# wbw520/scouter

Hardware: AMD Instinct MI355X
Metric: images/sec training step (resnest26d+xSlot, 224^2, bs70) (higher is better)
Workload: dtype f32; 1 GPU; BASELINE configs[1]: ImageNet-10 resnest26d + positive xSlot, channel 2048, T=3, to_k_layer 3, power 2, 224x224, per-GPU batch 70, random init, AdamW lr 1e-4; precision=fp32, activation_storage=fp32, register_split_bf16x3_layers=16, global_batch=70, parallelism=dp1, step=zero_grad+fwd+loss+bwd(+allreduce)+adamw, launch=eager

## Files before the change

include/scouter_hip.h:

```cpp
#ifndef SCOUTER_HIP_H
#define SCOUTER_HIP_H
#include <stddef.h>
#ifdef __cplusplus
extern "C" {
#endif

#define SC_OK 0
#define SC_ERR_ARG (-1)
#define SC_ERR_LAUNCH (-2)
#define SC_ERR_UNSUPPORTED (-3)
#define SC_ERR_WORKSPACE (-4)

int scouter_abi_version(void);
const char* scouter_last_error(void);

int scouter_set_switch(const char* name, int value);
int scouter_get_switch(const char* name);

int scouter_resize_normalize_u8_f32(const unsigned char* const* srcs, const int* hw, unsigned char* tmp,
                                    const long* tmp_off, const float* lut, float* out, int B, int C, int max_h, int max_w,
                                    int out_h, int out_w, void* stream);

void scouter_prof_enable(int on);
int scouter_prof_collect(char* buf, int cap);
// ... 291 lines not shown
int scouter_conv2d_x3_tile(long M, int N, int tile_hint);
int scouter_conv2d_x3_partial_rows(long M, int N, int tile_hint);
int scouter_conv2d_x3_halo_partial_rows(int groups);
int scouter_conv2d_fwd_x3(const float* x, const void* w_planes_fwd, const float* bias, const float* addend, float* y,
                          double* bn_partial, int B, int H, int W, int Cin, int Cout, int kh, int kw, int pad, int groups,
                          int relu, int tile_hint, void* stream);
int scouter_conv2d_dgrad_x3_bnbwd(const float* dy, const void* w_planes_dgrad, const float* addend, float* dx, int B,
                                  int H, int W, int Cin, int Cout, int kh, int kw, int pad, int groups, int tile_hint,
                                  const void* relu_mask, const float* x1, const float* saved1, double* part1,
                                  const float* x2, const float* saved2, double* part2, void* stream);

size_t scouter_conv2d_wgrad_x3_workspace_bytes(int B, int H, int W, int Cin, int Cout, int plan_hint);
int scouter_conv2d_wgrad_x3(const float* x, const float* dy, float* dw, int B, int H, int W, int Cin, int Cout,
                            int plan_hint, void* ws, size_t ws_bytes, void* stream);

size_t scouter_bn_fold_row_bytes(void);
int scouter_bn_fold_multi(const void* table, int nrows, long total, void* stream);
int scouter_sa_gate_fwd_f32(const float* gap, const float* w1, const float* b1, const float* w2, const float* b2, float* a,
                            int B, int Cp, int A, void* stream);

int scouter_iadd_i64(long* p, long n, long v, void* stream);

int scouter_adamw_chunk_bytes(void);
int scouter_adamw_step_f32(const void* chunk_table, int nchunks, const float* grads, float* exp_avg,
                           float* exp_avg_sq, float lr, float beta1, float beta2, float eps, float weight_decay,
                           int step, void* stream);
int scouter_adamw_step_dev_f32(const void* chunk_table, int nchunks, const float* grads, float* exp_avg,
                               float* exp_avg_sq, const float* dyn, float beta1, float beta2, float eps,
                               float weight_decay, void* stream);

// ... 5 lines not shown
```

scouter_amd/csrc/abi_core.hip:

```cpp
#include "common.h"

#include <stdarg.h>
#include <stdlib.h>
#include <atomic>
#include <map>
#include <mutex>
#include <vector>

#define SCOUTER_ABI_VERSION 1

static thread_local char g_err[512] = "";
static thread_local hipError_t g_lds_err = hipSuccess;

void sc_set_error(const char* fmt, ...) {
    va_list ap;
    va_start(ap, fmt);
    vsnprintf(g_err, sizeof(g_err), fmt, ap);
    va_end(ap);
}

int sc_check_launch(const char* what) {
    hipError_t e = hipGetLastError();
    if (e == hipSuccess) e = g_lds_err;
    g_lds_err = hipSuccess;
    if (e != hipSuccess) {
        sc_set_error("%s: launch failed: %s", what, hipGetErrorString(e));
        return SC_ERR_LAUNCH;
    }
    return SC_OK;
}

extern "C" int scouter_abi_version(void) { return SCOUTER_ABI_VERSION; }
extern "C" const char* scouter_last_error(void) { return g_err; }

static const char* const g_switch_names[SC_SW_COUNT] = {"xwt", "bwt", "bhalo", "xslot_small", "xslot_bwd_halves",
                                                         "xslot_bwd_scratch", "pwp_bn", "pwp_resident"};
struct SwitchTable {
    std::atomic<int> v[SC_SW_COUNT] = {};
    SwitchTable() {
        static const char* const flags[] = {"SCOUTER_XWT", "SCOUTER_BWT", "SCOUTER_BHALO", "SCOUTER_XSLOT_SMALL",
                                            "SCOUTER_XSLOT_BWD_HALVES", "SCOUTER_XSLOT_BWD_SCRATCH"};
        for (int i = 0; i <= SC_SW_XSLOT_BWD_SCRATCH; ++i) {
            const int def = i != SC_SW_XSLOT_BWD_SCRATCH;
            const char* e = getenv(flags[i]);
            v[i] = e && e[0] == '1' - def ? !def : def;
        }
        int bn = 0, r = 0;
        const char* e = getenv("SCOUTER_PWP_PLAN_DEV");
        if (e && sscanf(e, "%d,%d", &bn, &r) == 2 && bn > 0 && r > 0) { v[SC_SW_PWP_BN] = bn; v[SC_SW_PWP_RESIDENT] = r; }
    }
};
static SwitchTable& switch_table() {
    static SwitchTable t;
    return t;
}
int sc_switch(ScSwitch s) { return switch_table().v[s].load(std::memory_order_relaxed); }

static int switch_index(const char* name) {
    for (int i = 0; name && i < SC_SW_COUNT; ++i)
        if (strcmp(name, g_switch_names[i]) == 0) return i;
    sc_set_error("unknown switch '%s'", name ? name : "(null)");
// ... 81 lines not shown
```

scouter_amd/csrc/common.h:

```cpp
#pragma once
#include <hip/hip_runtime.h>
#include <stdint.h>
#include <stdio.h>
#include <string.h>

#define SC_OK 0
#define SC_ERR_ARG (-1)
#define SC_ERR_LAUNCH (-2)
#define SC_ERR_UNSUPPORTED (-3)
#define SC_ERR_WORKSPACE (-4)

typedef float f32x4 __attribute__((ext_vector_type(4)));
typedef float f32x16 __attribute__((ext_vector_type(16)));

void sc_set_error(const char* fmt, ...);
int sc_check_launch(const char* what);

enum ScSwitch { SC_SW_XWT, SC_SW_BWT, SC_SW_BHALO, SC_SW_XSLOT_SMALL, SC_SW_XSLOT_BWD_HALVES, SC_SW_XSLOT_BWD_SCRATCH,
                SC_SW_PWP_BN, SC_SW_PWP_RESIDENT, SC_SW_COUNT };
int sc_switch(ScSwitch s);

void sc_dyn_lds(const void* kern, size_t bytes);

#define SC_REQUIRE(cond, ...)                 \
    do {                                      \
        if (!(cond)) {                        \
            sc_set_error(__VA_ARGS__);        \
            return SC_ERR_ARG;                \
        }                                     \
    } while (0)

#define SC_UNSUPPORTED(cond, ...)             \
    do {                                      \
        if (!(cond)) {                        \
// ... 160 lines not shown
```

scouter_amd/csrc/conv_common.h:

```cpp
#pragma once
#include "common.h"

struct ConvGeom {
    int B, H, W, C;
    int Ho, Wo;
    int N;
    int R, S, stride, pad, groups;
    int Cg, Ng;
    long M;
    int wrow, wtap;
    double inv_hw;
    float inv_wo, inv_ho;
};

inline int sc_conv_out(int in, int k, int s, int p) { return (in + 2 * p - k) / s + 1; }

inline bool sc_pixels_ok(int B, int H, int W) {
    return B > 0 && H > 0 && W > 0 && H <= (1 << 24) && W <= (1 << 24) && (long)B * H <= (1L << 36) / W;
}
inline bool sc_conv_args_ok(int B, int H, int W, int Cin, int Cout, int kh, int kw, int stride, int pad, int groups) {
    const int lim = 1 << 16;
    return kh > 0 && kw > 0 && kh < lim && kw < lim && stride > 0 && pad >= 0 && pad < lim && sc_pixels_ok(B, H, W) &&
           sc_pixels_ok(B, H + 2 * pad, W + 2 * pad) && Cin > 0 && Cout > 0 && Cin <= (1 << 20) && Cout <= (1 << 20) && groups > 0 &&
           Cin % groups == 0 && Cout % groups == 0 && (long)(Cin / groups) * Cout < (1L << 31) && H + 2 * pad >= kh &&
// ... 42 lines not shown
__device__ __forceinline__ int fast_div(int n, float inv) { return (int)(((float)n + 0.5f) * inv); }


__device__ __forceinline__ void wgrad_block_coords(int& tile, int& split) {
    const int T = gridDim.x, S = gridDim.y, S8 = S & ~7;
    const int L = blockIdx.x + T * blockIdx.y;
    tile = blockIdx.x;
    split = blockIdx.y;
    if (L < T * S8) {
        const int xcd = L & 7, idx = L >> 3;
        split = xcd + 8 * (idx / T);
        tile = idx % T;
    }
}

void sc_launch_slab_reduce(const float* part, float* dst, long n, int splits, long slab, hipStream_t st);

struct BnBwdFuse {
    const unsigned long long* mask;
    const float* x1; const float* sv1; double* part1;
    const float* x2; const float* sv2; double* part2;
    int io;
};

bool sc_xhalo_ok(const ConvGeom& g);
int sc_xhalo_partial_rows(int groups);
void sc_launch_xhalo(bool dgrad, const float* a, const void* w_planes, long w_plane_elems, const float* addend, float* dst,
                     double* bn_part, const ConvGeom& g, int relu, hipStream_t st, const BnBwdFuse& fz);

template <int NR>
struct EpiPre { f32x4 add[NR], x1[NR], x2[NR]; bool on; };
// ... 361 lines not shown
```

scouter_amd/csrc/conv_igemm.hip:

```cpp
#include "conv_common.h"
#include "conv_wgrad_bf16.h"
#include "conv_wgrad_taps.h"
#include "conv_wgrad_taps_x3.h"
#include "conv_wgrad_taps_bf16.h"
#include "conv_pw_persist.h"
#include "conv_pw_persist_x3.h"

#include <stdlib.h>
#include <type_traits>

#ifdef IGEMM_STAMPS
__device__ long long* g_igemm_stamps = nullptr;
extern "C" int scouter_dev_set_igemm_stamps(void* p) {
    return (int)hipMemcpyToSymbol(HIP_SYMBOL(g_igemm_stamps), &p, sizeof(p));
}
#define IG_STAMP(k) if (g_igemm_stamps && threadIdx.x == 0) { asm volatile("s_waitcnt lgkmcnt(0)" ::: "memory"); g_igemm_stamps[8L * blockIdx.x + (k)] = (long long)wall_clock64(); }
#else
#define IG_STAMP(k)
#endif

constexpr int BK = 32;
constexpr int LDK = BK + 4;

template <int BM, int BN, bool B_KC>
// ... 520 lines not shown
        for (; k + 96 < splits; k += 128) {
#pragma unroll
            for (int u = 0; u < 4; ++u) s4[u] += *(const f32x4*)(part + (long)(k + 32 * u) * slab + i);
        }
        for (; k < splits; k += 32) s4[0] += *(const f32x4*)(part + (long)k * slab + i);
    }
    red[lane][q] = (s4[0] + s4[1]) + (s4[2] + s4[3]);
    __syncthreads();
    if (lane == 0 && i < n) {
        f32x4 s = red[0][q];
        for (int k = 1; k < 32; ++k) s += red[k][q];
        *(f32x4*)(dst + i) = s;
    }
}

void sc_launch_slab_reduce(const float* part, float* dst, long n, int splits, long slab, hipStream_t st) {
    hipLaunchKernelGGL(slab_reduce_kernel, dim3(sc_cdiv(n / 4, 8)), dim3(256), 0, st, part, dst, n, splits, slab);
}

template <int BM, int BN, int WM, int WN, bool DGRAD, bool STRIDED, bool PW>
static void launch_igemm_s(const float* src, const float* w, const float* bias, const float* addend, float* dst,
                           double* bn_part, const ConvGeom& g, int relu, hipStream_t st, const BnBwdFuse& fz) {
    const int mtiles = sc_cdiv(g.M, BM), ntiles = g.Ng / BN;
    dim3 grid(mtiles * ntiles * g.groups);
    const ConvGeom gg = sc_with_reciprocals(g);
    if (DGRAD && fz.part1)
        hipLaunchKernelGGL((igemm_kernel<BM, BN, WM, WN, DGRAD, STRIDED, PW, DGRAD>), grid, dim3(256), 0, st, src, w, bias,
                           addend, dst, bn_part, gg, relu, mtiles, ntiles, fz);
    else
        hipLaunchKernelGGL((igemm_kernel<BM, BN, WM, WN, DGRAD, STRIDED, PW, false>), grid, dim3(256), 0, st, src, w, bias,
                           addend, dst, bn_part, gg, relu, mtiles, ntiles, fz);
}
// ... 348 lines not shown
extern "C" size_t scouter_conv2d_wgrad_workspace_bytes(int B, int H, int W, int Cin, int Cout, int kh, int kw,
                                                       int stride, int pad, int groups, int plan_hint) {
    if (groups <= 0 || Cin % groups || Cout % groups) return 0;
    ConvGeom g = wgrad_geom(B, H, W, Cin, Cout, kh, kw, stride, pad, groups);
    WgradPlan p = wgrad_plan(g, plan_hint);
    size_t need = p.splits <= 1 ? 0 : (size_t)p.splits * kh * kw * g.Cg * Cout * sizeof(float);
    if (plan_hint < 0 && wgrad_taps_geom_ok(g)) {
        const long tiles = (long)(g.Ng / (g.Ng % 64 == 0 ? 64 : 32)) * groups;
        long want = 1024 / tiles;
        if (want < 1) want = 1;
        long chunks = (g.M + BK - 1) / BK, cps = (chunks + want - 1) / want;
        if (cps < 8) cps = 8;
        const long splits = (g.M + cps * BK - 1) / (cps * BK);
        const size_t nt = splits > 1 ? (size_t)splits * 9 * g.Cg * Cout * sizeof(float) : 0;
        if (nt > need) need = nt;
    }
    return need;
}

extern "C" int scouter_conv2d_wgrad_f32(const float* x, const float* dy, float* dw, int B, int H, int W, int Cin,
                                        int Cout, int kh, int kw, int stride, int pad, int groups, int plan_hint,
                                        void* ws, size_t ws_bytes, void* stream) {
    SC_REQUIRE(x && dy && dw && B > 0, "conv2d_wgrad: null pointer or empty shape");
    SC_REQUIRE(groups > 0 && Cin % groups == 0 && Cout % groups == 0, "conv2d_wgrad: channels not divisible by groups");
    ConvGeom g = wgrad_geom(B, H, W, Cin, Cout, kh, kw, stride, pad, groups);
    SC_UNSUPPORTED(wgrad_entry_ok(g), "conv2d_wgrad: per-group channels must be multiples of 32");
    if (plan_hint < 0 && wgrad_taps_geom_ok(g)) {
        const int bn = g.Ng % 64 == 0 ? 64 : 32;
        const int co_tiles = g.Ng / bn;
        const long tiles = (long)co_tiles * groups;
// ... 17 lines not shown
                                 4.0 * ((double)B * H * W * Cin + (double)g.M * Cout));
                auto kern = bn == 64 ? xwgrad_taps_kernel<64> : xwgrad_taps_kernel<32>;
                sc_dyn_lds((const void*)kern, xlds);
                hipLaunchKernelGGL(kern, dim3((unsigned)tiles, (unsigned)splits), dim3(256), xlds, st, x, dy, out, g, co_tiles,
                                   pps, slab_t);
            } else {
                ScProfScope prof("wgrad_taps", st, 2.0 * g.M * Cout * g.Cg * 9,
                                 4.0 * ((double)B * H * W * Cin + (double)g.M * Cout));
                auto kern = bn == 64 ? wgrad_taps_kernel<64> : wgrad_taps_kernel<32>;
                sc_dyn_lds((const void*)kern, lds);
                hipLaunchKernelGGL(kern, dim3((unsigned)tiles, (unsigned)splits), dim3(256), lds, st, x, dy, out, g, co_tiles,
                                   pps, slab_t);
            }
            int rc = sc_check_launch("conv2d_wgrad_taps");
            if (rc) return rc;
            if (splits > 1) {
                ScProfScope prof2("slab_reduce", st, 0, 4.0 * (double)slab_t * (splits + 1));
                hipLaunchKernelGGL(slab_reduce_kernel, dim3(sc_cdiv(slab_t / 4, 8)), dim3(256), 0, st, (const float*)ws,
                                   dw, slab_t, splits, slab_t);
                rc = sc_check_launch("conv2d_wgrad_taps_reduce");
            }
            return rc;
        }
    }
    WgradPlan p = wgrad_plan(g, plan_hint);
    const long slab = (long)kh * kw * g.Cg * Cout;
    const size_t need = p.splits > 1 ? (size_t)p.splits * slab * sizeof(float) : 0;
    if (need > ws_bytes || (need && !ws)) {
        sc_set_error("conv2d_wgrad: workspace too small (%zu < %zu bytes)", ws_bytes, need);
        return SC_ERR_WORKSPACE;
    }
    hipStream_t st = (hipStream_t)stream;
    float* out = p.splits > 1 ? (float*)ws : dw;
    dim3 grid((unsigned)p.tiles, (unsigned)p.splits);
    static char wname[9][24];
    static const int wb[9][2] = {{128, 128}, {128, 64}, {128, 32}, {64, 128}, {64, 64}, {64, 32}, {32, 128}, {32, 64}, {32, 32}};
// ... 18 lines not shown
                               p.ci_tiles, p.co_tiles, p.pix_per_split, slab);                                     \
    } while (0)
    if (p.bm == 128 && p.bn == 128) WG(128, 128, 64, 64);
    else if (p.bm == 128 && p.bn == 64) WG(128, 64, 64, 32);
    else if (p.bm == 128 && p.bn == 32) WG(128, 32, 32, 32);
    else if (p.bm == 64 && p.bn == 128) WG(64, 128, 32, 64);
    else if (p.bm == 64 && p.bn == 64) WG(64, 64, 32, 32);
    else if (p.bm == 64 && p.bn == 32) WG(64, 32, 32, 32);
    else if (p.bm == 32 && p.bn == 128) WG(32, 128, 32, 32);
    else if (p.bm == 32 && p.bn == 64) WG(32, 64, 32, 32);
    else WG(32, 32, 32, 32);
#undef WG
    }
    rc = sc_check_launch("conv2d_wgrad");
    if (rc) return rc;
    if (p.splits > 1) {
        const long n = slab;
        ScProfScope prof2("slab_reduce", st, 0, 4.0 * (double)slab * (p.splits + 1));
        hipLaunchKernelGGL(slab_reduce_kernel, dim3(sc_cdiv(n / 4, 8)), dim3(256), 0, st, (const float*)ws, dw, n,
                           p.splits, slab);
        rc = sc_check_launch("conv2d_wgrad_reduce");
    }
    return rc;
}

extern "C" int scouter_conv2d_wgrad_bf16_io(const void* x, const void* dy, float* dw, int B, int H, int W, int Cin,
                                            int Cout, int kh, int kw, int stride, int pad, int groups, int plan_hint,
                                            void* ws, size_t ws_bytes, int io, void* stream) {
    SC_REQUIRE(x && dy && dw && B > 0, "conv2d_wgrad_bf16: null pointer or empty shape");
    SC_REQUIRE((io & ~(SC_IO_X_BF16 | SC_IO_R_BF16)) == 0, "conv2d_wgrad_bf16: unsupported io bits %d (x and dy may be bf16)", io);
    const bool xb = (io & SC_IO_X_BF16) != 0, db = (io & SC_IO_R_BF16) != 0;
    SC_REQUIRE(groups > 0 && Cin % groups == 0 && Cout % groups == 0, "conv2d_wgrad_bf16: channels not divisible by groups");
    ConvGeom g = wgrad_geom(B, H, W, Cin, Cout, kh, kw, stride, pad, groups);
    const int mode = wgrad_same_mode(g, 64);
    SC_UNSUPPORTED(wgrad_bf16_geom_ok(g), "conv2d_wgrad_bf16: shape not covered by the bf16 kernel");
    if (plan_hint < 0 && bwt_geom_ok(g, io)) {
        const int bn = g.Ng % 64 == 0 ? 64 : 32;
// ... 8 lines not shown
        const long slab_t = (long)9 * g.Cg * Cout;
        const size_t need_t = splits > 1 ? (size_t)splits * slab_t * sizeof(float) : 0;
        if (sc_switch(SC_SW_BWT) && need_t <= ws_bytes && (!need_t || ws)) {
            hipStream_t st = (hipStream_t)stream;
            float* out = splits > 1 ? (float*)ws : dw;
            const size_t blds = bwgrad_taps_lds_bytes(bn);
            {
            ScProfScope prof("bwgrad_taps<bf16>", st, 2.0 * g.M * Cout * g.Cg * 9, 2.0 * ((double)B * H * W * Cin + (double)g.M * Cout));
            auto kern = bn == 64 ? bwgrad_taps_kernel<64> : bwgrad_taps_kernel<32>;
            sc_dyn_lds((const void*)kern, blds);
            hipLaunchKernelGGL(kern, dim3((unsigned)tiles, (unsigned)splits), dim3(256), blds, st, (const unsigned short*)x,
                               (const unsigned short*)dy, out, g, co_tiles, pps, slab_t);
            }
            int rc = sc_check_launch("conv2d_wgrad_taps_bf16");
            if (rc) return rc;
            if (splits > 1) {
                ScProfScope prof2("slab_reduce", st, 0, 4.0 * (double)slab_t * (splits + 1));
                hipLaunchKernelGGL(slab_reduce_kernel, dim3(sc_cdiv(slab_t / 4, 8)), dim3(256), 0, st, (const float*)ws,
                                   dw, slab_t, splits, slab_t);
                rc = sc_check_launch("conv2d_wgrad_taps_bf16_reduce");
            }
            return rc;
        }
    }
    WgradPlan p = wgrad_plan(g, plan_hint, true, 64);
    const long slab = (long)kh * kw * g.Cg * Cout;
    const size_t need = p.splits > 1 ? (size_t)p.splits * slab * sizeof(float) : 0;
    if (need > ws_bytes || (need && !ws)) {
        sc_set_error("conv2d_wgrad_bf16: workspace too small (%zu < %zu bytes)", ws_bytes, need);
        return SC_ERR_WORKSPACE;
    }
    hipStream_t st = (hipStream_t)stream;
    float* out = p.splits > 1 ? (float*)ws : dw;
    dim3 grid((unsigned)p.tiles, (unsigned)p.splits);
    int rc;
    {
// ... 15 lines not shown
        else if (mode == 2) WGK((wgrad_bf16_kernel<BM_, BN_, WM_, WN_, 2, false, false>));                          \
        else if (xb && db) WGK((wgrad_bf16_kernel<BM_, BN_, WM_, WN_, 1, true, true>));                             \
        else if (xb) WGK((wgrad_bf16_kernel<BM_, BN_, WM_, WN_, 1, true, false>));                                  \
        else if (db) WGK((wgrad_bf16_kernel<BM_, BN_, WM_, WN_, 1, false, true>));                                  \
        else WGK((wgrad_bf16_kernel<BM_, BN_, WM_, WN_, 1, false, false>));                                         \
    } while (0)
    if (p.bm == 128 && p.bn == 128) WGH(128, 128, 64, 64);
    else if (p.bm == 128 && p.bn == 64) WGH(128, 64, 64, 32);
    else if (p.bm == 64 && p.bn == 128) WGH(64, 128, 32, 64);
    else WGH(64, 64, 32, 32);
#undef WGH
#undef WGK
    }
    rc = sc_check_launch("conv2d_wgrad_bf16");
    if (rc) return rc;
    if (p.splits > 1) {
        ScProfScope prof2("slab_reduce", st, 0, 4.0 * (double)slab * (p.splits + 1));
        hipLaunchKernelGGL(slab_reduce_kernel, dim3(sc_cdiv(slab / 4, 8)), dim3(256), 0, st, (const float*)ws, dw, slab,
                           p.splits, slab);
        rc = sc_check_launch("conv2d_wgrad_bf16_reduce");
    }
    return rc;
}
extern "C" int scouter_conv2d_wgrad_bf16(const float* x, const float* dy, float* dw, int B, int H, int W, int Cin,
                                         int Cout, int kh, int kw, int stride, int pad, int groups, int plan_hint,
                                         void* ws, size_t ws_bytes, void* stream) {
    return scouter_conv2d_wgrad_bf16_io(x, dy, dw, B, H, W, Cin, Cout, kh, kw, stride, pad, groups, plan_hint, ws, ws_bytes,
                                        0, stream);
}
```

scouter_amd/csrc/conv_planes.hip:

```cpp
#include "conv_common.h"

#include <type_traits>

typedef __bf16 bf16x8 __attribute__((ext_vector_type(8)));

#define LDS_PTR(p) ((__attribute__((address_space(3))) void*)(p))

__device__ __forceinline__ void dma16(__amdgpu_buffer_rsrc_t rs, char* lds, unsigned voff, int soff) {
    __builtin_amdgcn_raw_ptr_buffer_load_lds(rs, LDS_PTR(lds), 16, voff, soff, 0, 0);
}

__device__ __forceinline__ f32x16 mfma_bf16p(bf16x8 a, bf16x8 b, f32x16 c) {
    return __builtin_amdgcn_mfma_f32_32x32x16_bf16(a, b, c, 0, 0, 0);
}

#define split3 split3_bf16

template <int NP>
__global__ __launch_bounds__(256) void split_planes_kernel(const float* __restrict__ x, unsigned short* __restrict__ p,
                                                           long n4, long plane_elems) {
    for (long i = (long)blockIdx.x * blockDim.x + threadIdx.x; i < n4; i += (long)gridDim.x * blockDim.x) {
        const f32x4 v = *(const f32x4*)(x + i * 4);
        u16x4 h, m, l;
#pragma unroll
// ... 1096 lines not shown
        if (nplanes == 3) {
            if (bm == 128 && bn == 128) PWG(128, 128, 3);
            else if (bm == 128) PWG(128, 64, 3);
            else if (bn == 128) PWG(64, 128, 3);
            else PWG(64, 64, 3);
        } else {
            if (bm == 128 && bn == 128) PWG(128, 128, 1);
            else if (bm == 128) PWG(128, 64, 1);
            else if (bn == 128) PWG(64, 128, 1);
            else PWG(64, 64, 1);
        }
#undef PWG
    }
    int rc = sc_check_launch("conv2d_wgrad_planes");
    if (rc) return rc;
    if (splits > 1) {
        ScProfScope prof2("slab_reduce", st, 0, 4.0 * (double)slab * (splits + 1));
        sc_launch_slab_reduce((const float*)ws, dw, slab, splits, slab, st);
        rc = sc_check_launch("conv2d_wgrad_planes_reduce");
    }
    return rc;
}
```

scouter_amd/csrc/conv_x3.hip:

```cpp
#include "conv_common.h"

#include <stdlib.h>
#include <type_traits>

typedef __bf16 xbf16x8 __attribute__((ext_vector_type(8)));
typedef unsigned short xu16x8 __attribute__((ext_vector_type(8)));

#define X3_LDS_PTR(p) ((__attribute__((address_space(3))) void*)(p))

#ifndef X3_ABLATE
#define X3_ABLATE 0
#endif

__device__ __forceinline__ void x3_dma16(__amdgpu_buffer_rsrc_t rs, char* lds, unsigned voff, int soff) {
    __builtin_amdgcn_raw_ptr_buffer_load_lds(rs, X3_LDS_PTR(lds), 16, voff, soff, 0, 0);
}
__device__ __forceinline__ f32x16 x3_mfma(xbf16x8 a, xbf16x8 b, f32x16 c) {
    return __builtin_amdgcn_mfma_f32_32x32x16_bf16(a, b, c, 0, 0, 0);
}

template <int BM, int BN, int NWM, int NWN, int MINB, bool DGRAD, bool CONV>
__global__ __launch_bounds__(NWM * NWN * 64, MINB) void xgemm_kernel(const float* __restrict__ a_f32,
                                                                       const unsigned short* __restrict__ w_planes, long w_plane_elems,
                                                                       const float* __restrict__ bias, const float* __restrict__ addend,
// ... 594 lines not shown
        return SC_ERR_WORKSPACE;
    }
    hipStream_t st = (hipStream_t)stream;
    float* out = p.splits > 1 ? (float*)ws : dw;
    int rc;
    {
        ScProfScope prof("xwgrad<bf16x3>", st, 2.0 * g.M * Cout * Cin, 4.0 * g.M * (Cin + Cout));
        constexpr int LDS = 2 * 3 * (128 + 128) * 40 * 2;
        auto kern = xwgrad_kernel<0>;
        sc_dyn_lds((const void*)kern, LDS);
        hipLaunchKernelGGL(kern, dim3((unsigned)p.tiles, (unsigned)p.splits), dim3(256), LDS, st, x, dy, out, g, p.ci_tiles,
                           p.co_tiles, p.pix_per_split, slab);
        rc = sc_check_launch("conv2d_wgrad_x3");
    }
    if (rc) return rc;
    if (p.splits > 1) {
        ScProfScope prof2("slab_reduce", st, 0, 4.0 * (double)slab * (p.splits + 1));
        sc_launch_slab_reduce((const float*)ws, dw, slab, p.splits, slab, st);
        rc = sc_check_launch("conv2d_wgrad_x3_reduce");
    }
    return rc;
}
```

scouter_amd/graph.py:

```python
import torch

from . import kernels as K


class GraphedTrainStep:

    def __init__(self, net, optimizer, warmup=3, preserve_state=True):
        self.preserve_state = bool(preserve_state)
        self.net = net
        self.model = net.module if hasattr(net, "module") else net
        self.optimizer = optimizer
        if not getattr(optimizer, "capturable", False):
            raise ValueError("GraphedTrainStep needs FusedAdamW(..., capturable=True)")
        self.warmup = max(int(warmup), 2)
        self.graph = None
        self._shape = None
        self.x = self.y = self.logp = self.stats = None
        self.replays = 0

    def _eager(self, x, y):
        model = self.model
        ddp = hasattr(self.net, "_issue_buffer_broadcast") and self.net._active and self.net.broadcast_buffers
        if ddp:
            self.net._issue_buffer_broadcast()
# ... 12 lines not shown
        self._one = torch.ones(1, dtype=torch.float32, device=dev)
        self.x = torch.empty_like(images, dtype=torch.float32).contiguous()
        self.y = torch.empty_like(labels, dtype=torch.int64)
        self.x.copy_(images)
        self.y.copy_(labels)
        self.model.train()
        snap = self._snapshot() if self.preserve_state else None
        s = torch.cuda.Stream(device=dev)
        s.wait_stream(torch.cuda.current_stream(dev))
        with torch.cuda.stream(s):
            for _ in range(self.warmup):
                self._eager(self.x, self.y)
        torch.cuda.current_stream(dev).wait_stream(s)
        torch.cuda.synchronize(dev)
        self.graph = torch.cuda.CUDAGraph()
        ws_before = set(K._ws)
        with torch.cuda.graph(self.graph):
            self.logp, self.stats = self._eager(self.x, self.y)
        self._pinned_ws = list(K._ws.values())
        sp = getattr(self.model, "_wsplitter", None)
        self._pinned_ws += sp.buffers() if sp is not None else []
        for key in set(K._ws) - ws_before:
            del K._ws[key]
        self._shape = (tuple(images.shape), tuple(labels.shape))
        for gi, _ in enumerate(self.optimizer.param_groups):
            st = self.optimizer.state.get("_flat_%d" % gi)
            if st is not None:
                st["step"] -= 1
        if snap is not None:
            self._restore(snap)
        return 0 if snap is not None else self.warmup

    def _named_state(self):
        named = dict(self.model.named_parameters())
# ... 54 lines not shown
```

scouter_amd/kernels.py:

```python
import contextlib
import os
import sys
import types

import torch

from . import _native

F32 = torch.float32
BF16 = torch.bfloat16
IO_X_BF16, IO_Y_BF16, IO_R_BF16 = 1, 2, 4
DGRAD_IO_ADDEND, DGRAD_IO_DY, DGRAD_IO_DX = 4, 8, 16
_ws = {}


_raw_stream = getattr(torch._C, "_cuda_getCurrentRawStream", None)


def _stream():
    if _raw_stream is not None:
        return _raw_stream(torch.cuda.current_device())
    return torch.cuda.current_stream().cuda_stream


# ... 47 lines not shown
    if not t.is_contiguous():
        raise RuntimeError("scouter_amd: %s must be contiguous" % name)


def _p(t):
    return None if t is None else t.data_ptr()


def workspace(nbytes, device):
    key = (device.type, device.index, _stream() if device.type == "cuda" else 0)
    w = _ws.get(key)
    if w is None or w.numel() < nbytes:
        w = torch.empty(max(int(nbytes), 1 << 20), dtype=torch.uint8, device=device)
        _ws[key] = w
    return w


def hwio(weight):
    v = weight.permute(2, 3, 1, 0)
    if not v.is_contiguous():
        with torch.no_grad():
            weight.data = weight.data.permute(2, 3, 1, 0).contiguous().permute(3, 2, 0, 1)
        v = weight.permute(2, 3, 1, 0)
    return v


def oihw_view(flat, cout, cin_g, kh, kw):
    return flat.view(kh, kw, cin_g, cout).permute(3, 2, 0, 1)


# ... 84 lines not shown
    if t is not None:
        return t
    _tile_cands[key] = tuple(c for c in candidates if c < 0 or launch(c, dry=True))
    if AUTOTUNE == "0":
        _tile_cache[key] = -1
        return -1
    if AUTOTUNE != "1":
        t = _table_choice(key, launch)
        if t >= 0 and t not in candidates:
            t = -1
        _tile_cache[key] = t
        return t
    best, best_ms = -1, None
    ev0, ev1 = torch.cuda.Event(enable_timing=True), torch.cuda.Event(enable_timing=True)
    torch.cuda.synchronize()
    for cand in candidates:
        if not launch(cand, dry=True):
            continue
        launch(cand)
        ms = None
        for _ in range(2 if TUNE_REPS > 3 else 1):
            ev0.record()
            for _ in range(TUNE_REPS):
                launch(cand)
            ev1.record()
            ev1.synchronize()
            m = ev0.elapsed_time(ev1)
            ms = m if ms is None else min(ms, m)
        if best_ms is None or ms < best_ms:
            best, best_ms = cand, ms
    _tile_cache[key] = best
    _record_choice(key, best)
    return best


class BnBwdFuse:
    __slots__ = ("mask", "entries", "parts", "rows")

    def __init__(self, mask, entries):
        assert 1 <= len(entries) <= 2
        self.mask, self.entries = mask, entries
        self.parts, self.rows = None, 0

    @property
    def applied(self):
# ... 494 lines not shown

def x3_wgrad_ok(cin, cout):
    return bool(ask("wgrad_x3_ok", 1, 8, 8, cin, cout))


def conv2d_wgrad_x3(x, dy, dw_hwio, plan=None):
    _chk(x, "x"); _chk(dy, "dy"); _chk(dw_hwio, "dw")
    B, H, W, Cin = x.shape
    Cout = dy.shape[-1]
    assert tuple(dw_hwio.shape) == (1, 1, Cin, Cout) and tuple(dy.shape[:3]) == (B, H, W)
    L = _native.lib()

    def launch(pl, dry=False):
        if dry:
            return True
        ws = workspace(L.scouter_conv2d_wgrad_x3_workspace_bytes(B, H, W, Cin, Cout, pl), x.device)
        _native.check(L.scouter_conv2d_wgrad_x3(_p(x), _p(dy), _p(dw_hwio), B, H, W, Cin, Cout, pl, _p(ws), ws.numel(),
                                                _stream()), "conv2d_wgrad_x3")
        return True
    if plan is None:
        plan = _pick_tile(("xwgrad", 3, B, H, W, Cin, Cout), launch, _X3_WGRAD_PLANS)
    launch(plan)
    return dw_hwio


def conv2d_wgrad_planes(xp, dyp, dw_hwio, pad, groups=1):
    nplanes, B, H, W, Cin = xp.shape
    kh, kw, cg, Cout = dw_hwio.shape
    L = _native.lib()

    def launch(plan, dry=False):
        if dry:
            return bool(ask("wgrad_planes_plan_ok", B, H, W, Cin, Cout, kh, kw, pad, groups, nplanes, plan))
        ws = workspace(L.scouter_conv2d_wgrad_planes_workspace_bytes(B, H, W, Cin, Cout, kh, kw, groups, plan), xp.device)
        _native.check(L.scouter_conv2d_wgrad_planes(_p(xp), _p(dyp), _p(dw_hwio), B, H, W, Cin, Cout, kh, kw, pad, groups,
                                                    nplanes, plan, _p(ws), ws.numel(), _stream()), "conv2d_wgrad_planes")
        return True

    launch(_pick_tile(("pwgrad", nplanes, B, H, W, Cin, Cout, kh, kw, pad, groups), launch, _PWGRAD_PLANS))
    return dw_hwio


_side = {}
_side_rr = [0]
SIDE_STREAMS = max(1, int(os.environ.get("SCOUTER_SIDE_STREAMS", "1")))
SIDE_STREAM_DEFAULT = os.environ.get("SCOUTER_SIDE_STREAM", "1") != "0"


def _side_priority(which):
# ... 51 lines not shown
    B, H, W, Cin = x.shape
    kh, kw, cg, Cout = dw_hwio.shape
    L = _native.lib()
    st = _stream()

    shape = (B, H, W, Cin, Cout, kh, kw, stride, pad, groups)
    bf16 = bool(precision == "bf16" and B * H * W >= BF16_MIN_PIXELS and ask("wgrad_kernel_ok", *shape, WGRAD_BF16))
    if (x.dtype != F32 or dy.dtype != F32) and not bf16:
        raise RuntimeError("scouter_amd: a bf16-stored activation / gradient needs the bf16-input weight-gradient kernel "
                           "(precision 'bf16', same-size stride-1 layer); got %s" % (tuple(x.shape),))

    def launch(plan, dry=False):
        if dry:
            return True
        need = L.scouter_conv2d_wgrad_workspace_bytes(B, H, W, Cin, Cout, kh, kw, stride, pad, groups, plan)
        ws = workspace(need, x.device)
        args = (_p(x), _p(dy), _p(dw_hwio), B, H, W, Cin, Cout, kh, kw, stride, pad, groups, plan, _p(ws), ws.numel())
        if bf16:
            _native.check(L.scouter_conv2d_wgrad_bf16_io(
                *args, (IO_X_BF16 if x.dtype == BF16 else 0) | (IO_R_BF16 if dy.dtype == BF16 else 0), st), "conv2d_wgrad")
        else:
            _native.check(L.scouter_conv2d_wgrad_f32(*args, st), "conv2d_wgrad")
        return True

    plan = _pick_tile(("wgrad", bf16, B, H, W, Cin, Cout, kh, kw, stride, pad, groups), launch, _WGRAD_PLANS)
    if not bf16 and get_switch("xwt") and ask("wgrad_kernel_ok", *shape, WGRAD_ROWS32):
        plan = -1
    if bf16 and get_switch("bwt") and wgrad_prerounds(*shape):
        if x.dtype != BF16:
            x = planes_split(x, 1)[0]
        if dy.dtype != BF16:
# ... 1049 lines not shown
```

scouter_amd/nn_hip.py:

```python
import math
import os
from collections import namedtuple

import torch
import torch.nn as nn

from . import kernels as K


class Act(nn.Module):

    def forward(self, x):
        raise RuntimeError("activation is fused; call the parent module")


GRAD_STORAGE_BF16 = os.environ.get("SCOUTER_BF16_GRADS", "1") != "0"

ConvRoute = namedtuple("ConvRoute", "fwd dgrad wgrad split_fwd split_dgrad planes_in planes_dy")
ConvCtx = namedtuple("ConvCtx", "x wd xp")
StemCtx = namedtuple("StemCtx", "x shape")


InferRoute = namedtuple("InferRoute", "fwd split")
FoldedConv = namedtuple("FoldedConv", "w b wf wt")
# ... 265 lines not shown
        col = K.im2col_nchw(x_nchw, self.kernel_size, self.stride, self.padding, self.kpad)
        wflat = K.hwio(self.weight).reshape(-1)
        wpad = K.pad_rows(wflat, wflat.numel(), self.kpad * self.out_channels).view(1, 1, self.kpad, self.out_channels)
        y = K.conv2d_fwd(col, wpad, None, addend, 1, 0, 1, relu, bn_stats, precision=self.precision)
        return y, (StemCtx(col, tuple(x_nchw.shape)) if save else None)

    def bwd(self, dy, ctx, need_dx=False, addend=None):
        dx = None
        if need_dx:
            if addend is not None:
                raise RuntimeError("StemConv2d.bwd: the image gradient takes no addend")
            dx = K.stem_dgrad(dy, K.hwio(self.weight), ctx.shape, self.kernel_size, self.stride, self.padding)
        if self._dw is not None:
            with K.side_stream(dy.device, ctx.x, dy, enabled=self.use_side_stream):
                dwpad = torch.empty((1, 1, self.kpad, self.out_channels), dtype=torch.float32, device=dy.device)
                K.conv2d_wgrad(ctx.x, dy, dwpad, precision=self.precision)
                n = self.kdim * self.out_channels
                K.axpby(dwpad.view(-1)[:n], None, 1.0, 0.0, out=self._dw.reshape(-1))
        return dx


class BatchNorm2d(nn.Module):

    def __init__(self, num_features, eps=1e-5, momentum=0.1):
        super().__init__()
        self.num_features, self.eps, self.momentum = num_features, eps, momentum
        self.weight = nn.Parameter(torch.ones(num_features))
        self.bias = nn.Parameter(torch.zeros(num_features))
        self.register_buffer("running_mean", torch.zeros(num_features))
        self.register_buffer("running_var", torch.ones(num_features))
        self.register_buffer("num_batches_tracked", torch.tensor(0, dtype=torch.long))
# ... 140 lines not shown
```

scouter_amd/sloter/slot_model.py:

```python
from collections import OrderedDict

import os

import torch
import torch.nn as nn

from .. import kernels as K
from ..nn_hip import Conv2d, FoldedConv, GradArena, StemConv2d
from ..timm.models import create_model
from .utils.position_encode import build_position_encoding
from .utils.slot_attention import SlotAttention

BF16_STORAGE_DEFAULT = os.environ.get("SCOUTER_BF16_STORAGE", "1") != "0"
SPLIT_ASYNC = os.environ.get("SCOUTER_SPLIT_ASYNC", "1") != "0"


class Identical(nn.Module):
    def forward(self, x):
        return x


def load_backbone(args):
    bone = create_model(args.model, pretrained=bool(getattr(args, "pre_trained", False)), num_classes=args.num_classes)
    if args.dataset == "MNIST":
# ... 354 lines not shown
                else:
                    runs.append([i, i + 1, count[i]])
            self._nbt_runs[key] = runs
        for lo, hi, c in runs:
            K.iadd_i64(self._nbt_flat[lo:hi], c)

    def _backward_impl(self, state, g_logp, g_loss, g_nll, g_term, need_input_grad=False):
        bctx, hstate = state
        arena = self.grad_arena()
        need = need_input_grad or self.backbone._first_trainable_stage() < 5
        last = self.backbone.last_fuse(bctx, need_input_grad) if need and self.use_slot else None
        dfeat = self._head_backward(hstate, g_logp, g_loss, g_nll, g_term, need_dfeat=need, post=last)
        done_hi = [arena.numel]

        def stage_done(name):
            lo = arena.first_offset("backbone." + name + ".")
            if lo is not None and lo < done_hi[0]:
                K.join_side_stream(arena.flat.device)
                for hook in self._grad_ready_hooks:
                    hook(arena, lo, done_hi[0])
                done_hi[0] = lo
        dx = None
        if need:
            dx = self.backbone.features_bwd(dfeat, bctx, stage_done if self._grad_ready_hooks else None, own=last,
                                            need_input_grad=need_input_grad)
        K.join_side_stream(arena.flat.device)
        if self._grad_ready_hooks and done_hi[0] > 0:
            for hook in self._grad_ready_hooks:
                hook(arena, 0, done_hi[0])
        arena.attach()
        for hook in self._post_backward_hooks:
            hook(arena)
        return dx

    def forward(self, x, target=None):
        train_graph = torch.is_grad_enabled() and (x.requires_grad or any(p.requires_grad for p in self.parameters()))
        if train_graph:
            if self._anchor is None or self._anchor.device != x.device:
                self._anchor = torch.zeros(1, device=x.device, requires_grad=True)
            self.grad_arena()
# ... 13 lines not shown
```

Before: 4833 images/sec.

## Defer split-K wgrad slab reductions and batch them into multi-row launches

Weight-gradient split-K reductions are no longer launched right after each wgrad kernel during backbone backward. Each partial-sum slab now gets its own region of a per-stream arena, and the reductions are queued and flushed at stage boundaries as one multi-row reduce kernel covering up to 16 tensors per launch. This aims to cut per-layer launch overhead and the serial tail of small reduce kernels. In exchange it needs more workspace memory (capped at 2 GB) and adds host-side bookkeeping, and graph capture has to pin the extra buffers.

```diff
diff --git a/include/scouter_hip.h b/include/scouter_hip.h
--- a/include/scouter_hip.h
+++ b/include/scouter_hip.h
@@ -329,6 +329,11 @@
 int scouter_conv2d_wgrad_x3(const float* x, const float* dy, float* dw, int B, int H, int W, int Cin, int Cout,
                             int plan_hint, void* ws, size_t ws_bytes, void* stream);
 
+int scouter_slab_defer_enable(int on);
+int scouter_slab_defer_flush(void* stream);
+int scouter_slab_defer_pending(void* stream, long* rows, size_t* bytes);
+int scouter_slab_sum_f32(const float* slabs, float* dst, long n, int splits, long stride, void* stream);
+
 size_t scouter_bn_fold_row_bytes(void);
 int scouter_bn_fold_multi(const void* table, int nrows, long total, void* stream);
 int scouter_sa_gate_fwd_f32(const float* gap, const float* w1, const float* b1, const float* w2, const float* b2, float* a,
diff --git a/scouter_amd/csrc/abi_core.hip b/scouter_amd/csrc/abi_core.hip
--- a/scouter_amd/csrc/abi_core.hip
+++ b/scouter_amd/csrc/abi_core.hip
@@ -34,7 +34,7 @@
 extern "C" const char* scouter_last_error(void) { return g_err; }
 
 static const char* const g_switch_names[SC_SW_COUNT] = {"xwt", "bwt", "bhalo", "xslot_small", "xslot_bwd_halves",
-                                                         "xslot_bwd_scratch", "pwp_bn", "pwp_resident"};
+                                                         "xslot_bwd_scratch", "pwp_bn", "pwp_resident", "slab_defer"};
 struct SwitchTable {
     std::atomic<int> v[SC_SW_COUNT] = {};
     SwitchTable() {
@@ -45,6 +45,8 @@
             const char* e = getenv(flags[i]);
             v[i] = e && e[0] == '1' - def ? !def : def;
         }
+        const char* d = getenv("SCOUTER_SLAB_DEFER");
+        v[SC_SW_SLAB_DEFER] = !(d && d[0] == '0');
         int bn = 0, r = 0;
         const char* e = getenv("SCOUTER_PWP_PLAN_DEV");
         if (e && sscanf(e, "%d,%d", &bn, &r) == 2 && bn > 0 && r > 0) { v[SC_SW_PWP_BN] = bn; v[SC_SW_PWP_RESIDENT] = r; }
diff --git a/scouter_amd/csrc/common.h b/scouter_amd/csrc/common.h
--- a/scouter_amd/csrc/common.h
+++ b/scouter_amd/csrc/common.h
@@ -17,7 +17,7 @@
 int sc_check_launch(const char* what);
 
 enum ScSwitch { SC_SW_XWT, SC_SW_BWT, SC_SW_BHALO, SC_SW_XSLOT_SMALL, SC_SW_XSLOT_BWD_HALVES, SC_SW_XSLOT_BWD_SCRATCH,
-                SC_SW_PWP_BN, SC_SW_PWP_RESIDENT, SC_SW_COUNT };
+                SC_SW_PWP_BN, SC_SW_PWP_RESIDENT, SC_SW_SLAB_DEFER, SC_SW_COUNT };
 int sc_switch(ScSwitch s);
 
 void sc_dyn_lds(const void* kern, size_t bytes);
diff --git a/scouter_amd/csrc/conv_common.h b/scouter_amd/csrc/conv_common.h
--- a/scouter_amd/csrc/conv_common.h
+++ b/scouter_amd/csrc/conv_common.h
@@ -80,7 +80,7 @@
     }
 }
 
-void sc_launch_slab_reduce(const float* part, float* dst, long n, int splits, long slab, hipStream_t st);
+int sc_slab_reduce(const float* part, float* dst, long n, int splits, long slab, hipStream_t st, const char* what);
 
 struct BnBwdFuse {
     const unsigned long long* mask;
diff --git a/scouter_amd/csrc/conv_igemm.hip b/scouter_amd/csrc/conv_igemm.hip
--- a/scouter_amd/csrc/conv_igemm.hip
+++ b/scouter_amd/csrc/conv_igemm.hip
@@ -7,7 +7,9 @@
 #include "conv_pw_persist_x3.h"
 
 #include <stdlib.h>
+#include <mutex>
 #include <type_traits>
+#include <vector>
 
 #ifdef IGEMM_STAMPS
 __device__ long long* g_igemm_stamps = nullptr;
@@ -558,8 +560,135 @@
     }
 }
 
-void sc_launch_slab_reduce(const float* part, float* dst, long n, int splits, long slab, hipStream_t st) {
+#define SLAB_ROWS 16
+#define SLAB_CPT 4
+struct SlabRow { const float* part; float* dst; long n, stride; int splits, lg; };
+struct SlabRows { SlabRow r[SLAB_ROWS]; int first[SLAB_ROWS + 1]; };
+
+__global__ __launch_bounds__(256) void slab_reduce_rows_kernel(const SlabRows rows) {
+    __shared__ f32x4 red[SLAB_CPT][256];
+    int ri = 0;
+    while (ri + 1 < SLAB_ROWS && (int)blockIdx.x >= rows.first[ri + 1]) ++ri;
+    const float* __restrict__ part = rows.r[ri].part;
+    float* __restrict__ dst = rows.r[ri].dst;
+    const long n = rows.r[ri].n, slab = rows.r[ri].stride;
+    const int splits = rows.r[ri].splits, lg = rows.r[ri].lg;
+    const int cpb = 256 >> lg;
+    const int q = threadIdx.x & (cpb - 1), lane = threadIdx.x >> (8 - lg);
+    const long col0 = (long)((int)blockIdx.x - rows.first[ri]) * (SLAB_CPT * cpb);
+    const float* p[SLAB_CPT];
+    f32x4 s4[SLAB_CPT][4];
+#pragma unroll
+    for (int c = 0; c < SLAB_CPT; ++c) {
+        const long i = (col0 + c * cpb + q) * 4;
+        p[c] = part + (i < n ? i : 0);
+#pragma unroll
+        for (int u = 0; u < 4; ++u) s4[c][u] = f32x4{0.f, 0.f, 0.f, 0.f};
+    }
+    int k = lane;
+    for (; k + 96 < splits; k += 128) {
+#pragma unroll
+        for (int u = 0; u < 4; ++u)
+#pragma unroll
+            for (int c = 0; c < SLAB_CPT; ++c) s4[c][u] += *(const f32x4*)(p[c] + (long)(k + 32 * u) * slab);
+    }
+    for (; k < splits; k += 32) {
+#pragma unroll
+        for (int c = 0; c < SLAB_CPT; ++c) s4[c][0] += *(const f32x4*)(p[c] + (long)k * slab);
+    }
+#pragma unroll
+    for (int c = 0; c < SLAB_CPT; ++c) red[c][threadIdx.x] = (s4[c][0] + s4[c][1]) + (s4[c][2] + s4[c][3]);
+    __syncthreads();
+    const int L = 1 << lg;
+    for (int o = threadIdx.x; o < SLAB_CPT * cpb; o += 256) {
+        const int c = o >> (8 - lg), oq = o & (cpb - 1);
+        const long i = (col0 + c * cpb + oq) * 4;
+        if (i < n) {
+            f32x4 s = red[c][oq];
+            for (int l = 1; l < L; ++l) s += red[c][l * cpb + oq];
+            *(f32x4*)(dst + i) = s;
+        }
+    }
+}
+
+struct SlabPending { hipStream_t st; std::vector<SlabRow> rows; };
+static std::mutex g_slab_mu;
+static std::vector<SlabPending> g_slab_pending;
+static thread_local int g_slab_defer = 0;
+
+int sc_slab_reduce(const float* part, float* dst, long n, int splits, long slab, hipStream_t st, const char* what) {
+    if (g_slab_defer) {
+        int lg = 0;
+        while ((1 << lg) < (splits < 32 ? splits : 32)) ++lg;
+        std::lock_guard<std::mutex> lk(g_slab_mu);
+        SlabPending* pd = nullptr;
+        for (auto& x : g_slab_pending) if (x.st == st) pd = &x;
+        if (!pd) { g_slab_pending.push_back(SlabPending{st, {}}); pd = &g_slab_pending.back(); }
+        pd->rows.push_back(SlabRow{part, dst, n, slab, splits, lg});
+        return SC_OK;
+    }
+    ScProfScope prof("slab_reduce", st, 0, 4.0 * (double)n * (splits + 1));
     hipLaunchKernelGGL(slab_reduce_kernel, dim3(sc_cdiv(n / 4, 8)), dim3(256), 0, st, part, dst, n, splits, slab);
+    return sc_check_launch(what);
+}
+
+extern "C" int scouter_slab_defer_enable(int on) {
+    const int was = g_slab_defer;
+    g_slab_defer = on != 0;
+    return was;
+}
+
+extern "C" int scouter_slab_defer_pending(void* stream, long* rows, size_t* bytes) {
+    std::lock_guard<std::mutex> lk(g_slab_mu);
+    long nr = 0;
+    size_t nb = 0;
+    for (auto& x : g_slab_pending)
+        if (x.st == (hipStream_t)stream) {
+            nr = (long)x.rows.size();
+            for (auto& r : x.rows) nb += (size_t)r.splits * r.stride * sizeof(float);
+        }
+    if (rows) *rows = nr;
+    if (bytes) *bytes = nb;
+    return SC_OK;
+}
+
+extern "C" int scouter_slab_defer_flush(void* stream) {
+    hipStream_t st = (hipStream_t)stream;
+    std::vector<SlabRow> todo;
+    {
+        std::lock_guard<std::mutex> lk(g_slab_mu);
+        for (auto& x : g_slab_pending) if (x.st == st) todo.swap(x.rows);
+    }
+    for (size_t at = 0; at < todo.size(); at += SLAB_ROWS) {
+        const int cnt = (int)(todo.size() - at < SLAB_ROWS ? todo.size() - at : SLAB_ROWS);
+        SlabRows a;
+        memset(&a, 0, sizeof(a));
+        double bytes = 0;
+        long total = 0;
+        for (int i = 0; i < cnt; ++i) {
+            const SlabRow& r = todo[at + i];
+            a.r[i] = r;
+            a.first[i] = (int)total;
+            total += sc_cdiv(r.n / 4, SLAB_CPT * (256 >> r.lg));
+            bytes += 4.0 * (double)r.n * (r.splits + 1);
+        }
+        SC_REQUIRE(total < (1L << 31), "slab_defer_flush: %ld workgroups in one launch", total);
+        for (int i = cnt; i <= SLAB_ROWS; ++i) a.first[i] = (int)total;
+        ScProfScope prof("slab_reduce", st, 0, bytes);
+        hipLaunchKernelGGL(slab_reduce_rows_kernel, dim3((unsigned)total), dim3(256), 0, st, a);
+        const int rc = sc_check_launch("slab_defer_flush");
+        if (rc) return rc;
+    }
+    return SC_OK;
+}
+
+extern "C" int scouter_slab_sum_f32(const float* slabs, float* dst, long n, int splits, long stride, void* stream) {
+    SC_REQUIRE(slabs && dst && n > 0 && splits >= 1, "slab_sum: null pointer or empty shape");
+    SC_REQUIRE(n % 4 == 0 && stride % 4 == 0 && stride >= n, "slab_sum: n = %ld and the slab stride %ld must be multiples of 4, stride >= n",
+               n, stride);
+    SC_REQUIRE(((uintptr_t)slabs | (uintptr_t)dst) % 16 == 0, "slab_sum: slabs and dst must be 16-byte aligned");
+    SC_REQUIRE(n / 4 < (1L << 31) * 8, "slab_sum: n = %ld is too long for one row", n);
+    return sc_slab_reduce(slabs, dst, n, splits, stride, (hipStream_t)stream, "slab_sum");
 }
 
 template <int BM, int BN, int WM, int WN, bool DGRAD, bool STRIDED, bool PW>
@@ -938,6 +1067,21 @@
         const long splits = (g.M + cps * BK - 1) / (cps * BK);
         const size_t nt = splits > 1 ? (size_t)splits * 9 * g.Cg * Cout * sizeof(float) : 0;
         if (nt > need) need = nt;
+    }
+    if (wgrad_bf16_geom_ok(g)) {
+        const WgradPlan pb = wgrad_plan(g, plan_hint, true, 64);
+        const size_t nb = pb.splits <= 1 ? 0 : (size_t)pb.splits * kh * kw * g.Cg * Cout * sizeof(float);
+        if (nb > need) need = nb;
+        if (plan_hint < 0 && bwt_geom_ok(g, SC_IO_X_BF16 | SC_IO_R_BF16)) {
+            const long tiles = (long)(g.Ng / (g.Ng % 64 == 0 ? 64 : 32)) * groups;
+            long want = 512 / tiles;
+            if (want < 1) want = 1;
+            long chunks = (g.M + BWT_CH - 1) / BWT_CH, cps = (chunks + want - 1) / want;
+            if (cps < 4) cps = 4;
+            const long splits = (g.M + cps * BWT_CH - 1) / (cps * BWT_CH);
+            const size_t nt = splits > 1 ? (size_t)splits * 9 * g.Cg * Cout * sizeof(float) : 0;
+            if (nt > need) need = nt;
+        }
     }
     return need;
 }
@@ -985,12 +1129,7 @@
             }
             int rc = sc_check_launch("conv2d_wgrad_taps");
             if (rc) return rc;
-            if (splits > 1) {
-                ScProfScope prof2("slab_reduce", st, 0, 4.0 * (double)slab_t * (splits + 1));
-                hipLaunchKernelGGL(slab_reduce_kernel, dim3(sc_cdiv(slab_t / 4, 8)), dim3(256), 0, st, (const float*)ws,
-                                   dw, slab_t, splits, slab_t);
-                rc = sc_check_launch("conv2d_wgrad_taps_reduce");
-            }
+            if (splits > 1) rc = sc_slab_reduce((const float*)ws, dw, slab_t, splits, slab_t, st, "conv2d_wgrad_taps_reduce");
             return rc;
         }
     }
@@ -1039,13 +1178,7 @@
     }
     rc = sc_check_launch("conv2d_wgrad");
     if (rc) return rc;
-    if (p.splits > 1) {
-        const long n = slab;
-        ScProfScope prof2("slab_reduce", st, 0, 4.0 * (double)slab * (p.splits + 1));
-        hipLaunchKernelGGL(slab_reduce_kernel, dim3(sc_cdiv(n / 4, 8)), dim3(256), 0, st, (const float*)ws, dw, n,
-                           p.splits, slab);
-        rc = sc_check_launch("conv2d_wgrad_reduce");
-    }
+    if (p.splits > 1) rc = sc_slab_reduce((const float*)ws, dw, slab, p.splits, slab, st, "conv2d_wgrad_reduce");
     return rc;
 }
 
@@ -1084,12 +1217,7 @@
             }
             int rc = sc_check_launch("conv2d_wgrad_taps_bf16");
             if (rc) return rc;
-            if (splits > 1) {
-                ScProfScope prof2("slab_reduce", st, 0, 4.0 * (double)slab_t * (splits + 1));
-                hipLaunchKernelGGL(slab_reduce_kernel, dim3(sc_cdiv(slab_t / 4, 8)), dim3(256), 0, st, (const float*)ws,
-                                   dw, slab_t, splits, slab_t);
-                rc = sc_check_launch("conv2d_wgrad_taps_bf16_reduce");
-            }
+            if (splits > 1) rc = sc_slab_reduce((const float*)ws, dw, slab_t, splits, slab_t, st, "conv2d_wgrad_taps_bf16_reduce");
             return rc;
         }
     }
@@ -1135,12 +1263,7 @@
     }
     rc = sc_check_launch("conv2d_wgrad_bf16");
     if (rc) return rc;
-    if (p.splits > 1) {
-        ScProfScope prof2("slab_reduce", st, 0, 4.0 * (double)slab * (p.splits + 1));
-        hipLaunchKernelGGL(slab_reduce_kernel, dim3(sc_cdiv(slab / 4, 8)), dim3(256), 0, st, (const float*)ws, dw, slab,
-                           p.splits, slab);
-        rc = sc_check_launch("conv2d_wgrad_bf16_reduce");
-    }
+    if (p.splits > 1) rc = sc_slab_reduce((const float*)ws, dw, slab, p.splits, slab, st, "conv2d_wgrad_bf16_reduce");
     return rc;
 }
 extern "C" int scouter_conv2d_wgrad_bf16(const float* x, const float* dy, float* dw, int B, int H, int W, int Cin,
diff --git a/scouter_amd/csrc/conv_planes.hip b/scouter_amd/csrc/conv_planes.hip
--- a/scouter_amd/csrc/conv_planes.hip
+++ b/scouter_amd/csrc/conv_planes.hip
@@ -1134,10 +1134,6 @@
     }
     int rc = sc_check_launch("conv2d_wgrad_planes");
     if (rc) return rc;
-    if (splits > 1) {
-        ScProfScope prof2("slab_reduce", st, 0, 4.0 * (double)slab * (splits + 1));
-        sc_launch_slab_reduce((const float*)ws, dw, slab, splits, slab, st);
-        rc = sc_check_launch("conv2d_wgrad_planes_reduce");
-    }
+    if (splits > 1) rc = sc_slab_reduce((const float*)ws, dw, slab, splits, slab, st, "conv2d_wgrad_planes_reduce");
     return rc;
 }
diff --git a/scouter_amd/csrc/conv_x3.hip b/scouter_amd/csrc/conv_x3.hip
--- a/scouter_amd/csrc/conv_x3.hip
+++ b/scouter_amd/csrc/conv_x3.hip
@@ -632,10 +632,6 @@
         rc = sc_check_launch("conv2d_wgrad_x3");
     }
     if (rc) return rc;
-    if (p.splits > 1) {
-        ScProfScope prof2("slab_reduce", st, 0, 4.0 * (double)slab * (p.splits + 1));
-        sc_launch_slab_reduce((const float*)ws, dw, slab, p.splits, slab, st);
-        rc = sc_check_launch("conv2d_wgrad_x3_reduce");
-    }
+    if (p.splits > 1) rc = sc_slab_reduce((const float*)ws, dw, slab, p.splits, slab, st, "conv2d_wgrad_x3_reduce");
     return rc;
 }
diff --git a/scouter_amd/graph.py b/scouter_amd/graph.py
--- a/scouter_amd/graph.py
+++ b/scouter_amd/graph.py
@@ -50,10 +50,13 @@
         torch.cuda.current_stream(dev).wait_stream(s)
         torch.cuda.synchronize(dev)
         self.graph = torch.cuda.CUDAGraph()
-        ws_before = set(K._ws)
+        ws_before, slab_before = set(K._ws), set(K._slab)
         with torch.cuda.graph(self.graph):
             self.logp, self.stats = self._eager(self.x, self.y)
         self._pinned_ws = list(K._ws.values())
+        self._pinned_ws += K.slab_buffers()
+        for key in set(K._slab) - slab_before:
+            del K._slab[key]
         sp = getattr(self.model, "_wsplitter", None)
         self._pinned_ws += sp.buffers() if sp is not None else []
         for key in set(K._ws) - ws_before:
diff --git a/scouter_amd/kernels.py b/scouter_amd/kernels.py
--- a/scouter_amd/kernels.py
+++ b/scouter_amd/kernels.py
@@ -1,6 +1,8 @@
 import contextlib
+import ctypes
 import os
 import sys
+import threading
 import types
 
 import torch
@@ -85,6 +87,115 @@
         w = torch.empty(max(int(nbytes), 1 << 20), dtype=torch.uint8, device=device)
         _ws[key] = w
     return w
+
+
+SLAB_DEFER_CAP = int(os.environ.get("SCOUTER_SLAB_DEFER_CAP_MB", "2048")) << 20
+_defer = threading.local()
+_slab = {}
+
+
+class _SlabBuf:
+    __slots__ = ("buf", "off", "want", "high", "flushes")
+
+    def __init__(self):
+        self.buf, self.off, self.want, self.high, self.flushes = None, 0, 0, 0, 0
+
+
+def slab_defer_active():
+    return getattr(_defer, "on", False)
+
+
+def _slab_set(on):
+    _defer.on = bool(on)
+    _native.lib().scouter_slab_defer_enable(int(on))
+
+
+@contextlib.contextmanager
+def slab_defer(enabled=True):
+    on = bool(enabled) and not slab_defer_active() and bool(get_switch("slab_defer"))
+    if not on:
+        yield False
+        return
+    _slab_set(True)
+    try:
+        yield True
+    finally:
+        _slab_set(False)
+        slab_defer_flush()
+
+
+@contextlib.contextmanager
+def slab_immediate():
+    was = slab_defer_active()
+    if was:
+        _slab_set(False)
+    try:
+        yield
+    finally:
+        if was:
+            _slab_set(True)
+
+
+def _slab_flush_one(key, sb):
+    sb.off = 0
+    sb.flushes += 1
+    _native.check(_native.lib().scouter_slab_defer_flush(key[2]), "slab_defer_flush")
+
+
+def slab_defer_flush(device=None):
+    n = 0
+    for key, sb in _slab.items():
+        if device is not None and (key[0], key[1]) != (device.type, device.index):
+            continue
+        if sb.off:
+            _slab_flush_one(key, sb)
+            n += 1
+        if sb.buf is not None and sb.want > sb.buf.numel() and sb.buf.numel() < SLAB_DEFER_CAP:
+            dev, size = sb.buf.device, min(sb.want, SLAB_DEFER_CAP)
+            sb.buf = None
+            if key[2] == _stream():
+                sb.buf = torch.empty(size, dtype=torch.uint8, device=dev)
+            else:
+                with torch.cuda.stream(torch.cuda.ExternalStream(key[2], device=dev)):
+                    sb.buf = torch.empty(size, dtype=torch.uint8, device=dev)
+        sb.want = 0
+    return n
+
+
+def slab_buffers():
+    return [sb.buf for sb in _slab.values() if sb.buf is not None]
+
+
+def slab_defer_stats():
+    return {k: (0 if sb.buf is None else sb.buf.numel(), sb.high, sb.flushes) for k, sb in _slab.items()}
+
+
+def slab_pending(stream=None):
+    rows, nbytes = ctypes.c_long(0), ctypes.c_size_t(0)
+    _native.check(_native.lib().scouter_slab_defer_pending(_stream() if stream is None else stream, ctypes.byref(rows),
+                                                           ctypes.byref(nbytes)), "slab_defer_pending")
+    return rows.value, nbytes.value
+
+
+def _wgrad_ws(nbytes, device):
+    if not nbytes or not slab_defer_active():
+        return workspace(nbytes, device)
+    key = (device.type, device.index, _stream())
+    sb = _slab.get(key)
+    if sb is None:
+        sb = _slab[key] = _SlabBuf()
+    need = (int(nbytes) + 255) // 256 * 256
+    sb.want += need
+    size = 0 if sb.buf is None else sb.buf.numel()
+    if sb.off and sb.off + need > min(size, SLAB_DEFER_CAP):
+        _slab_flush_one(key, sb)
+    if need > size:
+        sb.buf = None
+        sb.buf = torch.empty(need, dtype=torch.uint8, device=device)
+    ws = sb.buf[sb.off:sb.off + need]
+    sb.off += need
+    sb.high = max(sb.high, sb.off)
+    return ws
 
 
 def hwio(weight):
@@ -199,21 +310,22 @@
     best, best_ms = -1, None
     ev0, ev1 = torch.cuda.Event(enable_timing=True), torch.cuda.Event(enable_timing=True)
     torch.cuda.synchronize()
-    for cand in candidates:
-        if not launch(cand, dry=True):
-            continue
-        launch(cand)
-        ms = None
-        for _ in range(2 if TUNE_REPS > 3 else 1):
-            ev0.record()
-            for _ in range(TUNE_REPS):
-                launch(cand)
-            ev1.record()
-            ev1.synchronize()
-            m = ev0.elapsed_time(ev1)
-            ms = m if ms is None else min(ms, m)
-        if best_ms is None or ms < best_ms:
-            best, best_ms = cand, ms
+    with slab_immediate():
+        for cand in candidates:
+            if not launch(cand, dry=True):
+                continue
+            launch(cand)
+            ms = None
+            for _ in range(2 if TUNE_REPS > 3 else 1):
+                ev0.record()
+                for _ in range(TUNE_REPS):
+                    launch(cand)
+                ev1.record()
+                ev1.synchronize()
+                m = ev0.elapsed_time(ev1)
+                ms = m if ms is None else min(ms, m)
+            if best_ms is None or ms < best_ms:
+                best, best_ms = cand, ms
     _tile_cache[key] = best
     _record_choice(key, best)
     return best
@@ -738,7 +850,7 @@
     def launch(pl, dry=False):
         if dry:
             return True
-        ws = workspace(L.scouter_conv2d_wgrad_x3_workspace_bytes(B, H, W, Cin, Cout, pl), x.device)
+        ws = _wgrad_ws(L.scouter_conv2d_wgrad_x3_workspace_bytes(B, H, W, Cin, Cout, pl), x.device)
         _native.check(L.scouter_conv2d_wgrad_x3(_p(x), _p(dy), _p(dw_hwio), B, H, W, Cin, Cout, pl, _p(ws), ws.numel(),
                                                 _stream()), "conv2d_wgrad_x3")
         return True
@@ -756,7 +868,7 @@
     def launch(plan, dry=False):
         if dry:
             return bool(ask("wgrad_planes_plan_ok", B, H, W, Cin, Cout, kh, kw, pad, groups, nplanes, plan))
-        ws = workspace(L.scouter_conv2d_wgrad_planes_workspace_bytes(B, H, W, Cin, Cout, kh, kw, groups, plan), xp.device)
+        ws = _wgrad_ws(L.scouter_conv2d_wgrad_planes_workspace_bytes(B, H, W, Cin, Cout, kh, kw, groups, plan), xp.device)
         _native.check(L.scouter_conv2d_wgrad_planes(_p(xp), _p(dyp), _p(dw_hwio), B, H, W, Cin, Cout, kh, kw, pad, groups,
                                                     nplanes, plan, _p(ws), ws.numel(), _stream()), "conv2d_wgrad_planes")
         return True
@@ -838,7 +950,7 @@
         if dry:
             return True
         need = L.scouter_conv2d_wgrad_workspace_bytes(B, H, W, Cin, Cout, kh, kw, stride, pad, groups, plan)
-        ws = workspace(need, x.device)
+        ws = _wgrad_ws(need, x.device)
         args = (_p(x), _p(dy), _p(dw_hwio), B, H, W, Cin, Cout, kh, kw, stride, pad, groups, plan, _p(ws), ws.numel())
         if bf16:
             _native.check(L.scouter_conv2d_wgrad_bf16_io(
diff --git a/scouter_amd/nn_hip.py b/scouter_amd/nn_hip.py
--- a/scouter_amd/nn_hip.py
+++ b/scouter_amd/nn_hip.py
@@ -303,7 +303,8 @@
         if self._dw is not None:
             with K.side_stream(dy.device, ctx.x, dy, enabled=self.use_side_stream):
                 dwpad = torch.empty((1, 1, self.kpad, self.out_channels), dtype=torch.float32, device=dy.device)
-                K.conv2d_wgrad(ctx.x, dy, dwpad, precision=self.precision)
+                with K.slab_immediate():
+                    K.conv2d_wgrad(ctx.x, dy, dwpad, precision=self.precision)
                 n = self.kdim * self.out_channels
                 K.axpby(dwpad.view(-1)[:n], None, 1.0, 0.0, out=self._dw.reshape(-1))
         return dx
diff --git a/scouter_amd/sloter/slot_model.py b/scouter_amd/sloter/slot_model.py
--- a/scouter_amd/sloter/slot_model.py
+++ b/scouter_amd/sloter/slot_model.py
@@ -392,6 +392,9 @@
         done_hi = [arena.numel]
 
         def stage_done(name):
+            K.slab_defer_flush(arena.flat.device)
+            if not self._grad_ready_hooks:
+                return
             lo = arena.first_offset("backbone." + name + ".")
             if lo is not None and lo < done_hi[0]:
                 K.join_side_stream(arena.flat.device)
@@ -400,8 +403,8 @@
                 done_hi[0] = lo
         dx = None
         if need:
-            dx = self.backbone.features_bwd(dfeat, bctx, stage_done if self._grad_ready_hooks else None, own=last,
-                                            need_input_grad=need_input_grad)
+            with K.slab_defer(not need_input_grad):
+                dx = self.backbone.features_bwd(dfeat, bctx, stage_done, own=last, need_input_grad=need_input_grad)
         K.join_side_stream(arena.flat.device)
         if self._grad_ready_hooks and done_hi[0] > 0:
             for hook in self._grad_ready_hooks:
```

Measured after the change: 4858 images/sec (median of 6 runs). About the same (+0.5%).
